# Lakonik/SSDNeRF

Hardware: NVIDIA H100
Metric: rays/sec (128^2 render) & DDIM triplanes/sec (higher is better)
Workload: dtype fp16 tensor-core UNet (fp32 accumulate), fp32 renderer

## Files before the change

include/ssdnerf_b200.h:

```cpp
#ifndef SSDNERF_B200_H_
#define SSDNERF_B200_H_

#include <stdint.h>
#include <stddef.h>

#ifdef __cplusplus
extern "C" {
#endif

#define SSDNERF_API __attribute__((visibility("default")))

#define SSDNERF_OK 0
#define SSDNERF_ERR_CUDA (-1)
#define SSDNERF_ERR_ARG (-2)
#define SSDNERF_ERR_ARCH (-3)

SSDNERF_API const char* ssdnerf_last_error(void);
SSDNERF_API int ssdnerf_version(void);
SSDNERF_API int ssdnerf_compiled_arch(void);
SSDNERF_API unsigned long long ssdnerf_launch_count(void);

SSDNERF_API int ssdnerf_near_far_from_aabb(const float* rays_o, const float* rays_d, const float* aabb, uint32_t N, float min_near,
                               float* nears, float* fars, void* stream);
SSDNERF_API int ssdnerf_sph_from_ray(const float* rays_o, const float* rays_d, float radius, uint32_t N, float* coords, void* stream);
// ... 101 lines not shown
SSDNERF_API int ssdnerf_unpack_plane_grads(const float* grad_planes, const float* code, float reg_coef, uint32_t B, uint32_t Hp, uint32_t Wp,
                               int accumulate, float* grad_code, void* stream);
SSDNERF_API int ssdnerf_mse_render_loss(const float* image, const float* weights_sum, const float* target, uint64_t rays, float bg_color,
                            float coef_loss, float coef_grad, float* out_rgb , float* grad_image, float* grad_ws,
                            float* loss , void* stream);

SSDNERF_API size_t ssdnerf_density_workspace_bytes(uint32_t num_scenes, uint32_t grid_size);
SSDNERF_API int ssdnerf_density_update(int variant, const void* planes, uint32_t plane_h, uint32_t plane_w, const float* decoder_blob,
                           uint32_t num_scenes, uint32_t grid_size, float bound,
                           const float* jitter,
                           float decay, void* density_grid, int grid_is_half, void* workspace, void* stream);
SSDNERF_API int ssdnerf_density_pack(const void* density_grid, int grid_is_half, uint32_t num_scenes, uint32_t grid_size,
                         float density_thresh, uint8_t* bitfield, float* thresh_out ,
                         void* workspace, void* stream);

typedef struct ssdnerf_gemm_args {
    const void* a1; uint64_t a1_strides[3]; uint32_t k1;
    const void* a2; uint64_t a2_strides[3]; uint32_t k2;
    uint32_t d1, d2, d3, b1, b2, b3;
    uint32_t taps;
    const void* b; uint64_t b_strides[3]; uint32_t n, n_rows_b, bx2, bx3; uint32_t b_batched;
    uint32_t bn;
    float alpha;
    const float* bias_n;
    const void* residual;
    void* out; uint32_t out_f32; long long so1, so2, so3;
    float* qstats; uint32_t stats_hw;
    uint32_t algo;
    const int8_t* tap_offsets;
    uint32_t a_stride;
    uint32_t relu;
} ssdnerf_gemm_args;
SSDNERF_API int ssdnerf_gemm_f16(const ssdnerf_gemm_args* args, void* stream);

SSDNERF_API int ssdnerf_nchw_to_nhwc_f16(const float* x, uint32_t B, uint32_t C, uint32_t H, uint32_t W, uint32_t Cpad, void* out, void* stream);
SSDNERF_API int ssdnerf_gn_stats(const void* x1, uint32_t C1, const void* x2, uint32_t C2, uint32_t B, uint32_t HW, uint32_t groups,
                                 float* stats, void* stream);
SSDNERF_API int ssdnerf_gn_apply_q(const void* x1, uint32_t C1, const void* x2, uint32_t C2, uint32_t B, uint32_t HW, uint32_t groups,
                                   const float* q1, const float* q2, const float* gamma, const float* beta, const float* scale_shift,
                                   long long ss_batch_stride, float eps, int do_silu, void* out, void* stream);
SSDNERF_API int ssdnerf_gn_apply(const void* x1, uint32_t C1, const void* x2, uint32_t C2, uint32_t B, uint32_t HW, uint32_t groups,
                                 const float* stats, const float* gamma, const float* beta, const float* scale_shift,
                                 long long ss_batch_stride, float eps, int do_silu, void* out, void* stream);
SSDNERF_API int ssdnerf_flash_attn(const void* qkv, uint32_t B, uint32_t T, uint32_t heads, uint32_t ch, float scale, void* out, void* stream);
SSDNERF_API int ssdnerf_softmax_rows(const float* S, uint32_t rows, uint32_t T, void* P, void* stream);
SSDNERF_API int ssdnerf_transpose_v(const void* qkv, uint32_t B, uint32_t T, uint32_t heads, uint32_t ch, void* vt, void* stream);
SSDNERF_API int ssdnerf_ddim_update(float* x_t, const float* v, uint32_t B, uint32_t C, uint32_t H, uint32_t W, uint32_t Cv,
                                    const float* coef, const int* step_ptr, int clip, float clip_lo, float clip_hi, float* x0_out,
                                    void* next_in, uint32_t Cpad, void* stream);
SSDNERF_API int ssdnerf_ddpm_update(float* x_t, const float* v, uint32_t B, uint32_t C, uint32_t H, uint32_t W, uint32_t Cv,
                                    const float* coef, const int* step_ptr, const unsigned long long* seed_ptr, int clip, float clip_lo,
                                    float clip_hi, void* next_in, uint32_t Cpad, void* stream);
SSDNERF_API int ssdnerf_step_counter(int* step_ptr, int value, int set, void* stream);
SSDNERF_API int ssdnerf_select_row(const float* table, uint32_t row_elems, const int* step_ptr, float* dst, uint32_t copies, void* stream);

typedef struct ssdnerf_gn_bwd_args {
    const void* x1; uint32_t C1;
    const void* x2; uint32_t C2;
    uint32_t B, HW, groups;
    const float* stats; const float* stats2; int quad_stats;
    const float* gamma; const float* beta;
    const float* scale_shift; long long ss_batch_stride;
    float eps; int do_silu;
    const void* dy;
    const void* add;
    float* group_sums;
// ... 157 lines not shown
```

ssdnerf_b200/csrc/conv_row2.cu:

```cuda
#include "common.cuh"
#include "tc_common.cuh"
#include "conv_row_epilogue.cuh"
#include "../../include/ssdnerf_b200.h"
#include <cuda_fp16.h>

namespace ssdnerf {
using namespace tc;

constexpr int kRwThreads = 384;
constexpr int kRwRowSlot = 17 * 1024;
constexpr int kRwBSlot = kRwN * 128;
constexpr int kRwRows = 6, kRwBStages = 6;
constexpr size_t kRwSmem = (size_t)kRwRows * kRwRowSlot + (size_t)kRwBStages * kRwBSlot + 1024  + 256  +
                           256  + 512 ;

struct ConvRowParams {
    uint32_t B, H;
    const __half* x1; uint32_t C1;
    const __half* x2; uint32_t C2;
    long long xs1[3], xs2[3];
    const float* bias;
    const __half* residual;
    __half* out;
    float* qstats;
};

__global__ void __launch_bounds__(kRwThreads, 1)
k_conv_row2(const __grid_constant__ CUtensorMap mapB, const ConvRowParams p) {
    extern __shared__ uint8_t smem_raw[];
    uint8_t* smem = reinterpret_cast<uint8_t*>(((uintptr_t)smem_raw + 1023) & ~(uintptr_t)1023);
    uint8_t* sR = smem;
    uint8_t* sB = smem + kRwRows * kRwRowSlot;
    uint64_t* fullR = reinterpret_cast<uint64_t*>(sB + kRwBStages * kRwBSlot);
    uint64_t* emptyR = fullR + kRwRows;
    uint64_t* fullB = emptyR + kRwRows;
    uint64_t* emptyB = fullB + kRwBStages;
    float* qacc = reinterpret_cast<float*>(reinterpret_cast<uint8_t*>(fullR) + 256);
    float* sbias = qacc + 64;

    const int warp = threadIdx.x >> 5, lane = threadIdx.x & 31, wg = warp >> 2;
    const uint32_t tiles_per_img = p.H / 2, total_tiles = p.B * tiles_per_img;
    const uint32_t kc1 = p.C1 / 64, KC = (p.C1 + p.C2) / 64;
    const uint32_t tile0 = blockIdx.x, tstep = gridDim.x;
    const uint32_t my_tiles = tile0 < total_tiles ? (total_tiles - tile0 + tstep - 1) / tstep : 0;

    if (threadIdx.x == 0) {
        prefetch_tmap(&mapB);
        for (int i = 0; i < kRwRows; ++i) { mbar_init(&fullR[i], 4); mbar_init(&emptyR[i], 8); }
        for (int i = 0; i < kRwBStages; ++i) { mbar_init(&fullB[i], 1); mbar_init(&emptyB[i], 8); }
        fence_mbar_init();
    }
    for (int i = threadIdx.x; i < 64; i += kRwThreads) qacc[i] = 0.0f;
    for (int i = threadIdx.x; i < kRwN; i += kRwThreads) sbias[i] = p.bias ? __ldg(p.bias + i) : 0.0f;
    __syncthreads();
    pdl_trigger();
    pdl_wait();

    if (wg == 2) {
        setmaxnreg_dec<120>();
        const uint32_t lt = threadIdx.x - 256u;
        const uint32_t c8 = lt & 7u, p0 = lt >> 3;
        uint32_t idx = 0;
        for (uint32_t tile = tile0; tile < total_tiles; tile += tstep) {
            const uint32_t b = tile / tiles_per_img, y0 = (tile - b * tiles_per_img) * 2;
            for (uint32_t j = 0; j < KC; ++j) {
                const bool first = j < kc1;
                const __half* src = first ? p.x1 : p.x2;
                const long long xs0 = first ? p.xs1[0] : p.xs2[0], xs1 = first ? p.xs1[1] : p.xs2[1], xs2 = first ? p.xs1[2] : p.xs2[2];
                const uint32_t cl = (first ? j : j - kc1) * 64u + c8 * 8u;
                for (uint32_t r = 0; r < 4; ++r) {
                    const int y = (int)(y0 + r) - 1;
                    const bool row_ok = y >= 0 && y < (int)p.H;
                    const __half* rowp = src + (long long)b * xs2 + (long long)(row_ok ? y : 0) * xs1 + cl;
                    uint4 v[9];
#pragma unroll
                    for (int n = 0; n < 9; ++n) {
                        const int x = (int)(p0 + 16u * n) - 1;
                        v[n] = (row_ok && (unsigned)x < (unsigned)kRwW) ? __ldg(reinterpret_cast<const uint4*>(rowp + (long long)x * xs0))
                                                                       : make_uint4(0, 0, 0, 0);
                    }
                    const uint32_t slot = idx % kRwRows;
                    mbar_wait(&emptyR[slot], ((idx / kRwRows) & 1u) ^ 1u);
                    const uint32_t dst = smem_u32(sR + slot * kRwRowSlot);
#pragma unroll
                    for (int n = 0; n < 9; ++n) {
                        const uint32_t px = p0 + 16u * n;
                        if (px >= 130u) continue;
                        sts128(dst + px * 128u + ((c8 ^ (px & 7u)) << 4), v[n]);
                    }
                    __syncwarp();
                    if (lane == 0) mbar_arrive(&fullR[slot]);
                    ++idx;
                }
            }
        }
    } else {
        setmaxnreg_inc<192>();
        const uint32_t a = (uint32_t)wg, wq = (uint32_t)warp & 3u, cq = (uint32_t)lane & 3u;
        const uint32_t steps_per_tile = KC * 9u, total_steps = my_tiles * steps_per_tile;
        auto issue_w = [&](uint32_t L) {
            const uint32_t s = L % kRwBStages;
            if (L >= (uint32_t)kRwBStages) mbar_wait(&emptyB[s], ((L / kRwBStages) - 1u) & 1u);
            mbar_expect_tx(&fullB[s], (uint32_t)kRwBSlot);
            const uint32_t rem = L % steps_per_tile;
            tma_load_4d(sB + s * kRwBSlot, &mapB, &fullB[s], (int)((rem / 9u) * 64u), 0, (int)(rem % 9u), 0);
        };
        if (threadIdx.x == 0)
            for (uint32_t L = 0; L < total_steps && L < (uint32_t)kRwBStages; ++L) issue_w(L);
        auto release_row = [&](uint32_t ring) { if (lane == 0) mbar_arrive(&emptyR[ring % kRwRows]); };
        uint32_t m = 0, ridx = 0;
        const uint32_t lrow = wq * 16u + ((uint32_t)lane & 15u);
        const uint32_t lk = (uint32_t)lane >> 4;
// ... 48 lines not shown
#pragma unroll
                for (int h = 0; h < 2; ++h) {
#pragma unroll
                    for (int hh = 0; hh < 2; ++hh) {
                        const size_t o = (pix0 + 64u * h + wq * 16u + ((uint32_t)lane >> 2) + 8u * hh) * kRwN + ch;
                        float v0 = (h ? acc1 : acc0)[4 * i + 2 * hh] + b0, v1 = (h ? acc1 : acc0)[4 * i + 2 * hh + 1] + b1;
                        if (p.residual) { const float2 r = __half22float2(*reinterpret_cast<const __half2*>(p.residual + o)); v0 += r.x; v1 += r.y; }
                        *reinterpret_cast<__half2*>(p.out + o) = __floats2half2_rn(v0, v1);
                        su += v0 + v1; sq = fmaf(v0, v0, fmaf(v1, v1, sq));
                    }
                }
                if (p.qstats) {
                    frag_quad_reduce(su, sq);
                    if ((lane & ~2) == 0) { float* qa = qacc + (2 * i + (lane >> 1)) * 2; atomicAdd(qa, su); atomicAdd(qa + 1, sq); }
                }
            }
            if (p.qstats) {
                asm volatile("bar.sync 1, 256;" ::: "memory");
                if (threadIdx.x < 64) {
                    const float val = qacc[threadIdx.x];
                    if (val != 0.0f) atomicAdd(p.qstats + (size_t)b * 64 + threadIdx.x, val);
                    qacc[threadIdx.x] = 0.0f;
                }
                asm volatile("bar.sync 1, 256;" ::: "memory");
            }
        }
    }
    __syncthreads();
}

int make_map_4d_box(CUtensorMap* m, const void* base, uint64_t K, uint64_t e1, uint64_t e2, uint64_t e3, uint64_t s1, uint64_t s2, uint64_t s3,
                    uint32_t x1, uint32_t x2, uint32_t x3);

static int launch_row2(const CUtensorMap& mB, const ConvRowParams& p, int sms, cudaStream_t stream) {
    static DeviceOnce attr;
    if (attr.first()) {
        SSDNERF_CUDA_OK(cudaFuncSetAttribute(k_conv_row2, cudaFuncAttributeMaxDynamicSharedMemorySize, (int)kRwSmem));
    }
    const uint32_t total = p.B * (p.H / 2);
    SSDNERF_CUDA_OK(launch_pdl(k_conv_row2, dim3(total < (uint32_t)sms ? total : (uint32_t)sms), dim3(kRwThreads), kRwSmem, stream, mB, p));
    SSDNERF_LAUNCH_OK();
    return 0;
}

int conv_row2_launch(const ssdnerf_gemm_args* a, int sms, cudaStream_t stream) {
    if (((uintptr_t)a->a1 & 15u) || ((a->a1_strides[0] | a->a1_strides[1] | a->a1_strides[2]) & 15u) ||
        (a->a2 && (((uintptr_t)a->a2 & 15u) || ((a->a2_strides[0] | a->a2_strides[1] | a->a2_strides[2]) & 15u))) ||
        ((uintptr_t)a->out & 3u) || ((uintptr_t)a->residual & 3u))
        return set_error_msg(SSDNERF_ERR_ARG, "gemm: row-pair convolution needs 16-byte aligned inputs and strides, 4-byte aligned output / residual");
    ConvRowParams p{};
    p.B = a->d3; p.H = a->d2;
    p.x1 = (const __half*)a->a1; p.C1 = a->k1;
    p.x2 = (const __half*)a->a2; p.C2 = a->a2 ? a->k2 : 0;
    for (int i = 0; i < 3; ++i) { p.xs1[i] = (long long)(a->a1_strides[i] / 2); p.xs2[i] = a->a2 ? (long long)(a->a2_strides[i] / 2) : 0; }
    p.bias = a->bias_n; p.residual = (const __half*)a->residual; p.out = (__half*)a->out; p.qstats = a->qstats;
    const uint64_t ktot = (uint64_t)a->k1 + (a->a2 ? a->k2 : 0);
    CUtensorMap mB;
    if (int e = make_map_4d_box(&mB, a->b, ktot, a->n_rows_b ? a->n_rows_b : a->n, a->bx2 ? a->bx2 : 1, a->bx3 ? a->bx3 : 1, a->b_strides[0],
                                a->b_strides[1], a->b_strides[2], kRwN, 1, 1)) return e;
    return launch_row2(mB, p, sms, stream);
}

}
```

ssdnerf_b200/csrc/gemm_tc.cu:

```cuda
#include "common.cuh"
#include "tc_common.cuh"
#include "conv_row_epilogue.cuh"
#include "../../include/ssdnerf_b200.h"
#include <cuda_fp16.h>
#include <cstdio>

namespace ssdnerf {
using namespace tc;

constexpr int kGemmThreads = 384;
constexpr int kMaxBiasN = 2048;
constexpr int kBM = 128, kBK = 64;
constexpr int kABytes = kBM * kBK * 2;

struct GemmParams {
    uint32_t b1, b2, b3;
    uint32_t d1, d2, d3;
    uint32_t T1, T2, T3;
    uint32_t tiles_n;
    uint32_t taps;
    int8_t tap_ox[9], tap_oy[9];
    uint32_t a_stride;
    uint32_t kc1, kc2;
    uint32_t n_valid;
// ... 212 lines not shown
        cudaDriverEntryPointQueryResult qres;
        if (cudaGetDriverEntryPoint("cuTensorMapEncodeTiled", &p, cudaEnableDefault, &qres) != cudaSuccess || !p) return nullptr;
        fn = (PFN_encodeTiled)p;
    }
    return fn;
}

static int make_map_4d(CUtensorMap* m, const void* base, uint64_t K, uint64_t e1, uint64_t e2, uint64_t e3, uint64_t s1, uint64_t s2,
                       uint64_t s3, uint32_t x1, uint32_t x2, uint32_t x3, uint32_t trav = 1) {
    PFN_encodeTiled enc = get_encode();
    if (!enc) return set_error_msg(SSDNERF_ERR_CUDA, "cuTensorMapEncodeTiled entry point not found");
    if (((uintptr_t)base & 15u) || (s1 & 15u) || (s2 & 15u) || (s3 & 15u))
        return set_error_msg(SSDNERF_ERR_ARG, "gemm: TMA operands need 16-byte aligned base and strides");
    cuuint64_t dims[4] = {K, e1, e2, e3};
    cuuint64_t strides[3] = {s1, s2, s3};
    cuuint32_t box[4] = {64, x1 * trav, x2 * trav, x3};
    cuuint32_t estr[4] = {1, trav, trav, 1};
    const CUresult r = enc(m, CU_TENSOR_MAP_DATA_TYPE_FLOAT16, 4, const_cast<void*>(base), dims, strides, box, estr,
                           CU_TENSOR_MAP_INTERLEAVE_NONE, CU_TENSOR_MAP_SWIZZLE_128B, CU_TENSOR_MAP_L2_PROMOTION_L2_256B,
                           CU_TENSOR_MAP_FLOAT_OOB_FILL_NONE);
    if (r != CUDA_SUCCESS) {
        char buf[200];
        snprintf(buf, sizeof(buf), "cuTensorMapEncodeTiled failed (%d): dims {%llu,%llu,%llu,%llu} box {64,%u,%u,%u}", (int)r,
                 (unsigned long long)K, (unsigned long long)e1, (unsigned long long)e2, (unsigned long long)e3, x1, x2, x3);
        return set_error_msg(SSDNERF_ERR_CUDA, buf);
    }
    return 0;
}

int make_map_4d_box(CUtensorMap* m, const void* base, uint64_t K, uint64_t e1, uint64_t e2, uint64_t e3, uint64_t s1, uint64_t s2, uint64_t s3,
                    uint32_t x1, uint32_t x2, uint32_t x3) {
    return make_map_4d(m, base, K, e1, e2, e3, s1, s2, s3, x1, x2, x3);
}
int conv_row2_launch(const ssdnerf_gemm_args* a, int sms, cudaStream_t stream);

template <int BN, bool KT = false, bool RELU = false>
static int launch_gemm(const CUtensorMap& mA1, const CUtensorMap& mA2, const CUtensorMap& mB, const GemmParams& p, int sms,
                       cudaStream_t stream) {
    using Cfg = GemmCfg<BN>;
    static DeviceOnce attr;
    if (attr.first()) {
        SSDNERF_CUDA_OK(cudaFuncSetAttribute(k_gemm_tc<BN, KT, RELU>, cudaFuncAttributeMaxDynamicSharedMemorySize, (int)Cfg::kSmem));
    }
    const uint32_t total = p.T1 * p.T2 * p.T3 * p.tiles_n;
    cudaLaunchConfig_t cfg{};
    cfg.gridDim = dim3(total < (uint32_t)sms ? total : (uint32_t)sms);
    cfg.blockDim = dim3(kGemmThreads);
    cfg.dynamicSmemBytes = Cfg::kSmem;
    cfg.stream = stream;
    cudaLaunchAttribute at[1];
    at[0].id = cudaLaunchAttributeProgrammaticStreamSerialization;
    at[0].val.programmaticStreamSerializationAllowed = pdl_enabled() ? 1 : 0;
    cfg.attrs = at; cfg.numAttrs = 1;
    SSDNERF_CUDA_OK(cudaLaunchKernelEx(&cfg, k_gemm_tc<BN, KT, RELU>, mA1, mA2, mB, p));
    SSDNERF_LAUNCH_OK();
    return 0;
}

}

using namespace ssdnerf;

extern "C" int ssdnerf_gemm_f16(const ssdnerf_gemm_args* a, void* stream_) {
    cudaStream_t stream = (cudaStream_t)stream_;
    if (!a || !a->a1 || !a->b || !a->out) return set_error_msg(SSDNERF_ERR_ARG, "gemm: a1, b and out are required");
    const bool kt = a->algo == 3;
    if (kt) {
        if (a->k1 == 0 || a->k1 % 8 || (a->a2 && (a->k2 == 0 || a->k2 % 8)))
            return set_error_msg(SSDNERF_ERR_ARG, "gemm (narrow): K extents must be multiples of 8");
    } else if (a->k1 == 0 || a->k1 % 64 || a->k2 % 64) {
        return set_error_msg(SSDNERF_ERR_ARG, "gemm: K extents must be multiples of 64");
    }
    if (a->b1 * a->b2 * a->b3 != 128) return set_error_msg(SSDNERF_ERR_ARG, "gemm: b1*b2*b3 must be 128");
    if (a->taps < 1 || a->taps > 9) return set_error_msg(SSDNERF_ERR_ARG, "gemm: taps must be in [1, 9]");
    if (a->taps != 1 && a->taps != 9 && !a->tap_offsets) return set_error_msg(SSDNERF_ERR_ARG, "gemm: taps other than 1 / 9 need tap_offsets");
    if (a->taps > 1 && a->b_batched) return set_error_msg(SSDNERF_ERR_ARG, "gemm: conv taps and batched B are exclusive");
    if (a->a_stride > 2) return set_error_msg(SSDNERF_ERR_ARG, "gemm: a_stride must be 0 / 1 / 2");
    const uint32_t a_stride = a->a_stride == 2 ? 2u : 1u;
    if (a_stride == 2 && (a->b1 * 2 > 256 || a->b2 * 2 > 256)) return set_error_msg(SSDNERF_ERR_ARG, "gemm: stride-2 boxes exceed the 256-element TMA limit");
    if (a->n == 0 || a->d1 == 0 || a->d2 == 0 || a->d3 == 0) return 0;
    int dev = 0, sms = 0;
    SSDNERF_CUDA_OK(cudaGetDevice(&dev));
    SSDNERF_CUDA_OK(cudaDeviceGetAttribute(&sms, cudaDevAttrMultiProcessorCount, dev));
    if (a->algo != 1 && !kt && !a->relu && a->taps == 9 && !a->tap_offsets && a_stride == 1 && a->d1 == 128 && a->b1 == 128 && a->b2 == 1 && a->b3 == 1 && a->n == 128 && !a->out_f32 && !a->b_batched &&
        (a->d2 % 2) == 0 && a->alpha == 1.0f && (a->bn == 0 || a->bn == 128) && a->so1 == 128 && a->so2 == 128 * 128 &&
        a->so3 == (long long)a->d2 * 128 * 128 && (!a->qstats || a->stats_hw == 0) && (a->n_rows_b == 0 || a->n_rows_b >= 128))
        return ssdnerf::conv_row2_launch(a, sms, stream);
    if (a->algo == 2) return set_error_msg(SSDNERF_ERR_ARG, "gemm: algo 2 (row-pair convolution) needs taps 9, 128-pixel rows, 128 output channels, fp16 output");
    int bn = (int)a->bn;
    if (kt) {
        const int cand[6] = {256, 160, 80, 48, 40, 16};
        if (a->relu) {
            if (bn && bn != 16) return set_error_msg(SSDNERF_ERR_ARG, "gemm (narrow): relu needs bn 0 or 16");
            bn = 16;
        } else if (bn) {
            bool ok = false;
            for (int c : cand) ok |= c == bn;
            if (!ok) return set_error_msg(SSDNERF_ERR_ARG, "gemm (narrow): bn must be 16, 40, 48, 80, 160 or 256");
        } else {
            for (int c : cand) if (a->n % (uint32_t)c == 0) { bn = c; break; }
            if (!bn) {
                uint32_t best = 0xFFFFFFFFu;
                for (int c : cand) { const uint32_t w = div_up(a->n, (uint32_t)c) * (uint32_t)c; if (w < best) { best = w; bn = c; } }
            }
        }
    } else if (!bn) {
        const uint32_t tiles_m = div_up(a->d1, a->b1) * div_up(a->d2, a->b2) * div_up(a->d3, a->b3);
        double best = 1e30;
        const int cand[3] = {256, 128, 64};
        const double eff[3] = {1.0, 0.80, 0.50};
        for (int i = 0; i < 3; ++i) {
            if (cand[i] > 64 && (uint32_t)cand[i] / 2 >= a->n) continue;
            const uint32_t tiles = tiles_m * div_up(a->n, (uint32_t)cand[i]);
            const double t = (double)div_up(tiles, (uint32_t)sms) * cand[i] / eff[i];
            if (t < best) { best = t; bn = cand[i]; }
        }
    }
    if (!kt && bn != 64 && bn != 128 && bn != 256) return set_error_msg(SSDNERF_ERR_ARG, "gemm: bn must be 64, 128 or 256");

    GemmParams p{};
// ... 54 lines not shown
```

ssdnerf_b200/csrc/unet_glue.cu:

```cuda
#include "common.cuh"
#include "../../include/ssdnerf_b200.h"

namespace ssdnerf {

__device__ __forceinline__ void h8_to_f(const uint4& v, float* f) {
    const __half2* h = reinterpret_cast<const __half2*>(&v);
#pragma unroll
    for (int i = 0; i < 4; ++i) { const float2 t = __half22float2(h[i]); f[2 * i] = t.x; f[2 * i + 1] = t.y; }
}
__device__ __forceinline__ uint4 f_to_h8(const float* f) {
    uint4 o;
    __half2* h = reinterpret_cast<__half2*>(&o);
#pragma unroll
    for (int i = 0; i < 4; ++i) h[i] = __floats2half2_rn(f[2 * i], f[2 * i + 1]);
    return o;
}

__global__ void k_nchw_to_nhwc(const float* __restrict__ x, uint32_t B, uint32_t C, uint32_t HW, uint32_t Cpad, __half* __restrict__ out) {
    pdl_trigger();
    pdl_wait();
    const size_t i = threadIdx.x + (size_t)blockIdx.x * blockDim.x;
    const uint32_t cv = Cpad / 8;
    if (i >= (size_t)B * HW * cv) return;
    const uint32_t v = (uint32_t)(i % cv);
    const size_t bp = i / cv;
    const uint32_t pix = (uint32_t)(bp % HW), b = (uint32_t)(bp / HW);
    float f[8];
#pragma unroll
    for (int k = 0; k < 8; ++k) {
        const uint32_t c = v * 8 + k;
        f[k] = c < C ? __ldg(x + ((size_t)b * C + c) * HW + pix) : 0.0f;
    }
    reinterpret_cast<uint4*>(out)[i] = f_to_h8(f);
}

__global__ void __launch_bounds__(256) k_gn_stats(const __half* __restrict__ x1, uint32_t C1, const __half* __restrict__ x2, uint32_t C2,
                                                  uint32_t HW, uint32_t groups, uint32_t pix_per_block, float* __restrict__ stats) {
    pdl_trigger();
    pdl_wait();
    extern __shared__ float sm[];
    const uint32_t C = C1 + C2, cv = C / 8, cv1 = C1 / 8;
    const uint32_t b = blockIdx.y;
    for (uint32_t i = threadIdx.x; i < 2 * C; i += blockDim.x) sm[i] = 0.0f;
    __syncthreads();
    const uint32_t p0 = blockIdx.x * pix_per_block, p1 = min(p0 + pix_per_block, HW);
    {
        const uint32_t v = threadIdx.x % cv, lane_p = threadIdx.x / cv, pstep = blockDim.x / cv;
        float s[8], q[8];
#pragma unroll
// ... 25 lines not shown
    __syncthreads();
    const uint32_t cpg = C / groups;
    for (uint32_t g = threadIdx.x; g < groups; g += blockDim.x) {
        float s = 0.0f, q = 0.0f;
        for (uint32_t c = g * cpg; c < (g + 1) * cpg; ++c) { s += sm[c]; q += sm[C + c]; }
        atomicAdd(stats + ((size_t)b * groups + g) * 2, s);
        atomicAdd(stats + ((size_t)b * groups + g) * 2 + 1, q);
    }
}

__global__ void __launch_bounds__(256) k_gn_apply(const __half* __restrict__ x1, uint32_t C1, const __half* __restrict__ x2, uint32_t C2,
                                                  uint32_t HW, uint32_t groups, uint32_t pix_per_block, const float* __restrict__ stats,
                                                  const float* __restrict__ stats2, int quad_stats, const float* __restrict__ gamma, const float* __restrict__ beta,
                                                  const float* __restrict__ scale_shift, long long ss_batch_stride, float eps, int do_silu,
                                                  __half* __restrict__ out) {
    pdl_trigger();
    pdl_wait();
    const uint32_t C = C1 + C2, cv = C / 8, cv1 = C1 / 8;
    const uint32_t b = blockIdx.y;
    const uint32_t v = threadIdx.x % cv, lane_p = threadIdx.x / cv, pstep = blockDim.x / cv;
    const uint32_t cpg = C / groups;
    const float inv_n = 1.0f / ((float)HW * (float)cpg);
    const float* ss = scale_shift ? scale_shift + (size_t)b * ss_batch_stride : nullptr;
    float ga[8], be[8], sc[8], sh[8];
#pragma unroll
    for (int k = 0; k < 8; ++k) {
        const uint32_t c = v * 8 + k;
        ga[k] = __ldg(gamma + c); be[k] = __ldg(beta + c);
        sc[k] = ss ? 1.0f + __ldg(ss + c) : 1.0f; sh[k] = ss ? __ldg(ss + C + c) : 0.0f;
    }
    __shared__ float2 s_mr[64];
    if (threadIdx.x < groups) {
        const uint32_t g = threadIdx.x;
        float sm = 0.0f, sq = 0.0f;
        if (!quad_stats) {
            sm = __ldg(stats + ((size_t)b * groups + g) * 2); sq = __ldg(stats + ((size_t)b * groups + g) * 2 + 1);
        } else {
            const uint32_t q1n = C1 / 4, q2n = C2 / 4, nq = cpg / 4;
            for (uint32_t i = 0; i < nq; ++i) {
                const uint32_t qi = g * nq + i;
                const float2 t = __ldg(reinterpret_cast<const float2*>(qi < q1n ? stats + ((size_t)b * q1n + qi) * 2
                                                                                  : stats2 + ((size_t)b * q2n + (qi - q1n)) * 2));
                sm += t.x; sq += t.y;
            }
        }
        const float mean = sm * inv_n;
        s_mr[g] = make_float2(mean, rsqrtf(fmaxf(sq * inv_n - mean * mean, 0.0f) + eps));
    }
    __syncthreads();
    float a[8], bb[8];
#pragma unroll
    for (int k = 0; k < 8; ++k) {
        const float2 mr = s_mr[(v * 8 + k) / cpg];
        const float ak = mr.y * ga[k];
        const float bk = be[k] - mr.x * ak;
        a[k] = ak * sc[k]; bb[k] = fmaf(bk, sc[k], sh[k]);
    }
    const __half* src = v < cv1 ? x1 + (size_t)b * HW * C1 + v * 8 : x2 + (size_t)b * HW * C2 + (v - cv1) * 8;
    const uint32_t cs = v < cv1 ? C1 : C2;
    __half* dst = out + (size_t)b * HW * C + v * 8;
    const uint32_t p0 = blockIdx.x * pix_per_block, p1 = min(p0 + pix_per_block, HW);
    auto emit = [&](const uint4& r, uint32_t p) {
        float f[8];
        h8_to_f(r, f);
#pragma unroll
        for (int k = 0; k < 8; ++k) { float y = fmaf(f[k], a[k], bb[k]); f[k] = do_silu ? silu_f(y) : y; }
        *reinterpret_cast<uint4*>(dst + (size_t)p * C) = f_to_h8(f);
    };
    uint32_t p = p0 + lane_p;
    for (; p + 3 * pstep < p1; p += 4 * pstep) {
        uint4 r[4];
#pragma unroll
        for (int u = 0; u < 4; ++u) r[u] = __ldg(reinterpret_cast<const uint4*>(src + (size_t)(p + u * pstep) * cs));
#pragma unroll
        for (int u = 0; u < 4; ++u) emit(r[u], p + u * pstep);
    }
    for (; p < p1; p += pstep) emit(__ldg(reinterpret_cast<const uint4*>(src + (size_t)p * cs)), p);
}

__global__ void __launch_bounds__(256) k_softmax_rows(const float* __restrict__ S, uint32_t rows, uint32_t T, __half* __restrict__ P) {
    pdl_trigger();
    pdl_wait();
    const uint32_t warp = threadIdx.x >> 5, lane = threadIdx.x & 31;
    const uint32_t row = blockIdx.x * 8 + warp;
    if (row >= rows) return;
    const float4* src = reinterpret_cast<const float4*>(S + (size_t)row * T);
    const uint32_t nv = T / 4;
    float m = -INFINITY;
    for (uint32_t i = lane; i < nv; i += 32) { const float4 v = __ldg(src + i); m = fmaxf(m, fmaxf(fmaxf(v.x, v.y), fmaxf(v.z, v.w))); }
#pragma unroll
    for (int o = 16; o > 0; o >>= 1) m = fmaxf(m, __shfl_xor_sync(0xffffffffu, m, o));
    float sum = 0.0f;
    for (uint32_t i = lane; i < nv; i += 32) { const float4 v = __ldg(src + i); sum += __expf(v.x - m) + __expf(v.y - m) + __expf(v.z - m) + __expf(v.w - m); }
#pragma unroll
    for (int o = 16; o > 0; o >>= 1) sum += __shfl_xor_sync(0xffffffffu, sum, o);
    const float inv = 1.0f / sum;
    __half2* dst = reinterpret_cast<__half2*>(P + (size_t)row * T);
    for (uint32_t i = lane; i < nv; i += 32) {
        const float4 v = __ldg(src + i);
        dst[2 * i] = __floats2half2_rn(__expf(v.x - m) * inv, __expf(v.y - m) * inv);
        dst[2 * i + 1] = __floats2half2_rn(__expf(v.z - m) * inv, __expf(v.w - m) * inv);
// ... 187 lines not shown
```

ssdnerf_b200/unet.py:

```python
import math
from copy import deepcopy

import torch
import torch.nn as nn

from . import _lib as N
from . import unet_ops as U
from .registry import MODULES


_GN_GROUPS = [32]


def _gn(c):
    return nn.GroupNorm(_GN_GROUPS[0], c, eps=1e-5)


class _ResBlockParams(nn.Module):

    def __init__(self, cin, cout, emb_ch, dropout=0.0):
        super().__init__()
        self.conv_1 = nn.Sequential(_gn(cin), nn.SiLU(), nn.Conv2d(cin, cout, 3, padding=1))
        self.norm_with_embedding = nn.Module()
        self.norm_with_embedding.norm = _gn(cout)
# ... 331 lines not shown
        L, s = N.lib(), N.stream_ptr()
        ss = None
        if ss_off is not None:
            ss = N.c_void_p(self.ss_cur.data_ptr() + 4 * ss_off)
        if ((C1 + C2) // G) % 4 != 0 or q1 is None or (x2 is not None and q2 is None):
            self._legacy_idx += 1
            st = self._q(('legacy', self._legacy_idx), G * 4)
            N.check(L.ssdnerf_gn_stats(N.ptr(x1), N.c_u32(C1), N.ptr(x2), N.c_u32(C2), N.c_u32(B), N.c_u32(H * W), N.c_u32(G), N.ptr(st), s))
            N.check(L.ssdnerf_gn_apply(N.ptr(x1), N.c_u32(C1), N.ptr(x2), N.c_u32(C2), N.c_u32(B), N.c_u32(H * W), N.c_u32(G), N.ptr(st),
                                       N.ptr(gamma), N.ptr(beta), ss, N.c_longlong(self.ss_total), N.c_f32(1e-5), N.c_int(int(silu)),
                                       N.ptr(out), s))
            self._last_stats = (False, st, None)
            return out
        self._last_stats = (True, q1, q2)
        N.check(L.ssdnerf_gn_apply_q(N.ptr(x1), N.c_u32(C1), N.ptr(x2), N.c_u32(C2), N.c_u32(B), N.c_u32(H * W), N.c_u32(G), N.ptr(q1),
                                     N.ptr(q2), N.ptr(gamma), N.ptr(beta), ss, N.c_longlong(self.ss_total), N.c_f32(1e-5),
                                     N.c_int(int(silu)), N.ptr(out), s))
        return out

    def _res(self, d, x, skip, tag):
        (x, qx), (sk, qs) = x, (skip if skip is not None else (None, None))
        B, H, W, _ = x.shape
        cin, cout = d['cin'], d['cout']
        nw = self.narrow
        if 'ws' in d:
            sc = U.conv3x3_f16(x, d['ws'].unsqueeze(0), cout, bias=d['wsb'], x2=sk, taps=1, out=self._buf(('sc', H, cout), (B, H, W, cout)),
                               narrow=nw)
        else:
            if sk is not None:
                raise NotImplementedError('ResBlock with a skip concat but no shortcut convolution (cin + skip == cout) is not built')
            sc = x
        qh1 = self._q(('h1', tag), cout)
        qo = self._q(('res_out', tag), cout)
        a = self._gn(x, qx, sk, qs, d['g1'], d['b1'], self._buf(('a', H, cin), (B, H, W, cin)), True)
        st1 = self._last_stats
        h1 = U.conv3x3_f16(a, d['w1'], cout, bias=d['c1b'], out=self._buf(('h1', tag) if self.saving else ('h1', H, cout), (B, H, W, cout)),
                           qstats=qh1, narrow=nw)
        a2 = self._gn(h1, qh1, None, None, d['g2'], d['b2'], self._buf(('a2', H, cout), (B, H, W, cout)), True, self.ss_offsets[d['idx']])
        st2 = self._last_stats
        if self.saving:
            self._dropout(a2, d['idx'])
        out = U.conv3x3_f16(a2, d['w2'], cout, bias=d['c2b'], residual=sc, out=self._buf(('res_out', tag), (B, H, W, cout)), qstats=qo,
                            narrow=nw)
        if self.saving:
            self.tape.append(dict(kind='res', d=d, x=x, sk=sk, st1=st1, h1=h1, st2=st2, out=out, tag=tag))
        return out, qo

    def _attn(self, d, x, tag):
        x, qx = x
        B, H, W, c = x.shape
        T, heads = H * W, d['heads']
        ch = c // heads
        L, s = N.lib(), N.stream_ptr()
        xn = self._gn(x, qx, None, None, d['g'], d['b'], self._buf(('xn', T, c), (B, H, W, c)), False)
        st = self._last_stats
        qkv = U.linear_f16(xn.view(B * T, c), d['wqkv'], bias=d['bqkv'], n=3 * c,
                           out=self._buf(('qkv', tag) if self.saving else ('qkv', T, c), (B * T, 3 * c)), narrow=self.narrow)
        o = self._attn_core(qkv, B, T, c, heads, ('o', T, c))
        qo = self._q(('attn_out', tag), c) if T % 64 == 0 else None
        out = U.linear_f16(o.view(B * T, c), d['wproj'], bias=d['bproj'], residual=x.view(B * T, c), n=c,
                           out=self._buf(('attn_out', tag), (B * T, c)), qstats=qo, stats_hw=T, narrow=self.narrow).view(B, H, W, c)
        if self.saving:
            self.tape.append(dict(kind='attn', d=d, x=x, st=st, qkv=qkv.view(B, T, 3 * c), out=out, tag=tag))
        return out, qo

    def _attn_core(self, qkv, B, T, c, heads, out_key):
        ch = c // heads
        L, s = N.lib(), N.stream_ptr()
        if ch in (64, 128) and T % 64 == 0:
            return U.flash_attn(qkv.view(B, T, 3 * c), heads, 1.0 / math.sqrt(ch), out=self._buf(out_key, (B, T, c)))
        S = U.attn_scores(qkv.view(B, T, 3 * c), heads, scale=1.0 / math.sqrt(ch), out=self._buf(('S', T), (B, heads, T, T), torch.float32),
                          narrow=self.narrow)
        P = self._buf(('P', T), (B, heads, T, T))
        N.check(L.ssdnerf_softmax_rows(N.ptr(S), N.c_u32(B * heads * T), N.c_u32(T), N.ptr(P), s))
        vt = self._buf(('vt', T, c), (B, heads, ch, T))
        N.check(L.ssdnerf_transpose_v(N.ptr(qkv), N.c_u32(B), N.c_u32(T), N.c_u32(heads), N.c_u32(ch), N.ptr(vt), s))
# ... 252 lines not shown
```

ssdnerf_b200/unet_ops.py:

```python
import ctypes

import torch

from . import _lib as N

c_u64 = ctypes.c_uint64
c_ll = ctypes.c_longlong


class GemmArgs(ctypes.Structure):
    _fields_ = [
        ('a1', N.c_void_p), ('a1_strides', c_u64 * 3), ('k1', N.c_u32),
        ('a2', N.c_void_p), ('a2_strides', c_u64 * 3), ('k2', N.c_u32),
        ('d1', N.c_u32), ('d2', N.c_u32), ('d3', N.c_u32), ('b1', N.c_u32), ('b2', N.c_u32), ('b3', N.c_u32),
        ('taps', N.c_u32),
        ('b', N.c_void_p), ('b_strides', c_u64 * 3), ('n', N.c_u32), ('n_rows_b', N.c_u32), ('bx2', N.c_u32), ('bx3', N.c_u32),
        ('b_batched', N.c_u32),
        ('bn', N.c_u32), ('alpha', N.c_f32), ('bias_n', N.c_void_p), ('residual', N.c_void_p),
        ('out', N.c_void_p), ('out_f32', N.c_u32), ('so1', c_ll), ('so2', c_ll), ('so3', c_ll),
        ('qstats', N.c_void_p), ('stats_hw', N.c_u32), ('algo', N.c_u32),
        ('tap_offsets', N.c_void_p), ('a_stride', N.c_u32), ('relu', N.c_u32),
    ]


ALGO_NARROW = 3


def _launch(a):
    N.check(N.lib().ssdnerf_gemm_f16(ctypes.byref(a), N.stream_ptr()))


def _pad_rows(w, mult=64):
    n = w.shape[-2]
    pad = (-n) % mult
    if pad:
        w = torch.cat([w, w.new_zeros(*w.shape[:-2], pad, w.shape[-1])], dim=-2)
    return w


def pack_linear_weight(w, narrow=False):
    w = w.detach().reshape(w.shape[0], -1).half()
    assert w.shape[1] % (8 if narrow else 64) == 0, 'K must be a multiple of 64 (narrow: of 8)'
    return _pad_rows(w).contiguous()


def pack_conv_weight(w, cin_pad=None, narrow=False):
    cout, cin = w.shape[0], w.shape[1]
    m = 8 if narrow else 64
    cin_pad = cin_pad or ((cin + m - 1) // m * m)
    wp = w.detach().permute(2, 3, 0, 1).reshape(9, cout, cin).half()
    if cin_pad != cin:
        wp = torch.cat([wp, wp.new_zeros(9, cout, cin_pad - cin)], dim=-1)
    return _pad_rows(wp).contiguous()


# ... 18 lines not shown
    g.out, g.out_f32 = out.data_ptr(), int(out.dtype == torch.float32)
    g.so1, g.so2, g.so3 = out.stride(0), 0, 0
    if qstats is not None:
        g.qstats, g.stats_hw = qstats.data_ptr(), stats_hw
    if narrow:
        g.algo = ALGO_NARROW
    _launch(g)
    return out


def _conv_boxes(H, W, narrow=False):
    if narrow:
        return _conv_boxes_narrow(H, W)
    bw = min(W, 128)
    bh = min(H, 128 // bw)
    nb = 128 // (bw * bh)
    return bw, bh, nb


def _pow2_floor(v):
    return 1 << (max(int(v), 1).bit_length() - 1)


def _conv_boxes_narrow(H, W):
    bw = min(128, W & -W)
    bh = min(128 // bw, _pow2_floor(H))
    if 128 // (bw * bh) > 2:
        bw = min(128, 1 << (W - 1).bit_length())
        bh = min(128 // bw, 1 << (H - 1).bit_length())
    return bw, bh, 128 // (bw * bh)


def conv3x3_f16(x, wp, cout, bias=None, x2=None, residual=None, out=None, out_f32=False, taps=9, bn=0, qstats=None, algo=0, narrow=False,
                relu=False):
    N.require_cuda(x, wp)
    B, H, W, C1 = x.shape
    C2 = x2.shape[-1] if x2 is not None else 0
    assert x.is_contiguous() and (x2 is None or x2.is_contiguous())
    km = 8 if narrow else 64
    assert wp.shape[-1] == C1 + C2 and C1 % km == 0 and C2 % km == 0, (wp.shape, C1, C2)
    if narrow:
        algo = ALGO_NARROW
    if out is None:
        out = torch.empty(B, H, W, cout, dtype=torch.float32 if out_f32 else torch.float16, device=x.device)
    bw, bh, nb = _conv_boxes(H, W, narrow)
    g = GemmArgs()
    g.a1, g.k1 = x.data_ptr(), C1
    g.a1_strides = (c_u64 * 3)(C1 * 2, W * C1 * 2, H * W * C1 * 2)
    if x2 is not None:
        g.a2, g.k2 = x2.data_ptr(), C2
        g.a2_strides = (c_u64 * 3)(C2 * 2, W * C2 * 2, H * W * C2 * 2)
    g.d1, g.d2, g.d3, g.b1, g.b2, g.b3 = W, H, B, bw, bh, nb
    g.taps = taps
    ktot = C1 + C2
    rows = wp.shape[-2]
    g.b, g.n, g.n_rows_b, g.bx2, g.bx3 = wp.data_ptr(), cout, rows, taps, 1
    g.b_strides = (c_u64 * 3)(ktot * 2, rows * ktot * 2, taps * rows * ktot * 2)
    g.bn, g.alpha, g.algo = bn, 1.0, algo
    g.bias_n = bias.data_ptr() if bias is not None else None
    g.residual = residual.data_ptr() if residual is not None else None
    g.out, g.out_f32 = out.data_ptr(), int(out.dtype == torch.float32)
    co = out.shape[-1]
    g.so1, g.so2, g.so3 = co, W * co, H * W * co
    if qstats is not None:
        g.qstats, g.stats_hw = qstats.data_ptr(), 0
    g.relu = int(relu)
    _launch(g)
    return out


def conv3x3_s2_f16(x, wp, cout, bias=None, out=None, qstats=None, narrow=False):
    N.require_cuda(x, wp)
    B, H, W, C = x.shape
    assert x.is_contiguous() and H % 2 == 0 and W % 2 == 0 and wp.shape[-1] == C and C % (8 if narrow else 64) == 0
    Ho, Wo = H // 2, W // 2
    if out is None:
        out = torch.empty(B, Ho, Wo, cout, dtype=torch.float16, device=x.device)
    bw, bh, nb = _conv_boxes(Ho, Wo, narrow)
    g = GemmArgs()
    g.a1, g.k1 = x.data_ptr(), C
    g.a1_strides = (c_u64 * 3)(C * 2, W * C * 2, H * W * C * 2)
    g.d1, g.d2, g.d3, g.b1, g.b2, g.b3 = Wo, Ho, B, bw, bh, nb
    g.taps, g.a_stride = 9, 2
    rows = wp.shape[-2]
    g.b, g.n, g.n_rows_b, g.bx2, g.bx3 = wp.data_ptr(), cout, rows, 9, 1
    g.b_strides = (c_u64 * 3)(C * 2, rows * C * 2, 9 * rows * C * 2)
    g.bn, g.alpha, g.algo = 0, 1.0, ALGO_NARROW if narrow else 1
    g.bias_n = bias.data_ptr() if bias is not None else None
    g.out, g.out_f32 = out.data_ptr(), int(out.dtype == torch.float32)
    g.so1, g.so2, g.so3 = cout, Wo * cout, Ho * Wo * cout
    if qstats is not None:
        g.qstats, g.stats_hw = qstats.data_ptr(), 0
    _launch(g)
    return out


_UP_ROWS = {0: ((-1, (0,)), (0, (1, 2))), 1: ((0, (0, 1)), (1, (2,)))}


def pack_upconv_weight(w, narrow=False):
    w = w.detach().float()
# ... 247 lines not shown
```

Measured before the change: 97.93 million.

## Fuse GroupNorm+SiLU apply into the row-pair convolution loader

Adds a GroupNorm descriptor to the fp16 GEMM entry point. When it is given, the row-pair 3x3 conv's loader warps normalize, scale/shift and apply SiLU to each input vector before staging it in shared memory, so the resblock no longer writes and re-reads a separate normalized activation buffer. The unet glue routes the 128-wide, 128-channel resblocks through this path. The cost is extra per-channel coefficient loads and group-stat reductions inside the producer warps, which could slow the producer side of the pipeline.

```diff
diff --git a/include/ssdnerf_b200.h b/include/ssdnerf_b200.h
--- a/include/ssdnerf_b200.h
+++ b/include/ssdnerf_b200.h
@@ -157,6 +157,14 @@
     uint32_t relu;
 } ssdnerf_gemm_args;
 SSDNERF_API int ssdnerf_gemm_f16(const ssdnerf_gemm_args* args, void* stream);
+typedef struct ssdnerf_gn_desc {
+    const float* q1; const float* q2;
+    const float* gamma; const float* beta;
+    const float* scale_shift;
+    long long ss_batch_stride;
+    float eps; uint32_t groups;
+} ssdnerf_gn_desc;
+SSDNERF_API int ssdnerf_gemm_f16_gn(const ssdnerf_gemm_args* args, const ssdnerf_gn_desc* gn, void* stream);
 
 SSDNERF_API int ssdnerf_nchw_to_nhwc_f16(const float* x, uint32_t B, uint32_t C, uint32_t H, uint32_t W, uint32_t Cpad, void* out, void* stream);
 SSDNERF_API int ssdnerf_gn_stats(const void* x1, uint32_t C1, const void* x2, uint32_t C2, uint32_t B, uint32_t HW, uint32_t groups,
diff --git a/ssdnerf_b200/csrc/conv_row2.cu b/ssdnerf_b200/csrc/conv_row2.cu
--- a/ssdnerf_b200/csrc/conv_row2.cu
+++ b/ssdnerf_b200/csrc/conv_row2.cu
@@ -1,6 +1,7 @@
 #include "common.cuh"
 #include "tc_common.cuh"
 #include "conv_row_epilogue.cuh"
+#include "gn_apply.cuh"
 #include "../../include/ssdnerf_b200.h"
 #include <cuda_fp16.h>
 
@@ -23,8 +24,32 @@
     const __half* residual;
     __half* out;
     float* qstats;
+    const float* gq1; const float* gq2;
+    const float* gamma; const float* beta;
+    const float* ss; long long ss_stride;
+    float eps; uint32_t cpg;
 };
 
+__device__ __forceinline__ void loader_gn_coeffs(const ConvRowParams& p, uint32_t b, uint32_t c0, float* a, float* bb) {
+    const uint32_t C = p.C1 + p.C2, nq = p.cpg / 4;
+    const float* ss = p.ss ? p.ss + (size_t)b * p.ss_stride : nullptr;
+    float ga[8], be[8], sc[8], sh[8];
+#pragma unroll
+    for (int k = 0; k < 8; ++k) {
+        const uint32_t c = c0 + k;
+        ga[k] = __ldg(p.gamma + c); be[k] = __ldg(p.beta + c);
+        sc[k] = ss ? 1.0f + __ldg(ss + c) : 1.0f; sh[k] = ss ? __ldg(ss + C + c) : 0.0f;
+    }
+    const uint32_t g0 = c0 / p.cpg, g1 = (c0 + 7u) / p.cpg;
+    const float2 s0 = gn_quad_group_sums(p.gq1, p.gq2, p.C1 / 4, p.C2 / 4, b, g0, nq);
+    const float2 s1 = gn_quad_group_sums(p.gq1, p.gq2, p.C1 / 4, p.C2 / 4, b, g1, nq);
+    const float inv_n = 1.0f / ((float)(p.H * kRwW) * (float)p.cpg);
+    const float2 mr0 = gn_mean_rstd(s0, inv_n, p.eps), mr1 = gn_mean_rstd(s1, inv_n, p.eps);
+#pragma unroll
+    for (int k = 0; k < 8; ++k) gn_fold((c0 + k) / p.cpg == g0 ? mr0 : mr1, ga[k], be[k], sc[k], sh[k], a[k], bb[k]);
+}
+
+template <bool GN>
 __global__ void __launch_bounds__(kRwThreads, 1)
 k_conv_row2(const __grid_constant__ CUtensorMap mapB, const ConvRowParams p) {
     extern __shared__ uint8_t smem_raw[];
@@ -68,6 +93,8 @@
                 const __half* src = first ? p.x1 : p.x2;
                 const long long xs0 = first ? p.xs1[0] : p.xs2[0], xs1 = first ? p.xs1[1] : p.xs2[1], xs2 = first ? p.xs1[2] : p.xs2[2];
                 const uint32_t cl = (first ? j : j - kc1) * 64u + c8 * 8u;
+                float ga[8], gb[8];
+                if constexpr (GN) loader_gn_coeffs(p, b, j * 64u + c8 * 8u, ga, gb);
                 for (uint32_t r = 0; r < 4; ++r) {
                     const int y = (int)(y0 + r) - 1;
                     const bool row_ok = y >= 0 && y < (int)p.H;
@@ -78,6 +105,11 @@
                         const int x = (int)(p0 + 16u * n) - 1;
                         v[n] = (row_ok && (unsigned)x < (unsigned)kRwW) ? __ldg(reinterpret_cast<const uint4*>(rowp + (long long)x * xs0))
                                                                        : make_uint4(0, 0, 0, 0);
+                    }
+                    if constexpr (GN) {
+#pragma unroll
+                        for (int n = 0; n < 9; ++n)
+                            if (row_ok && (unsigned)((int)(p0 + 16u * n) - 1) < (unsigned)kRwW) v[n] = gn_transform_h8(v[n], ga, gb, true);
                     }
                     const uint32_t slot = idx % kRwRows;
                     mbar_wait(&emptyR[slot], ((idx / kRwRows) & 1u) ^ 1u);
@@ -192,18 +224,19 @@
 int make_map_4d_box(CUtensorMap* m, const void* base, uint64_t K, uint64_t e1, uint64_t e2, uint64_t e3, uint64_t s1, uint64_t s2, uint64_t s3,
                     uint32_t x1, uint32_t x2, uint32_t x3);
 
+template <bool GN>
 static int launch_row2(const CUtensorMap& mB, const ConvRowParams& p, int sms, cudaStream_t stream) {
     static DeviceOnce attr;
     if (attr.first()) {
-        SSDNERF_CUDA_OK(cudaFuncSetAttribute(k_conv_row2, cudaFuncAttributeMaxDynamicSharedMemorySize, (int)kRwSmem));
+        SSDNERF_CUDA_OK(cudaFuncSetAttribute(k_conv_row2<GN>, cudaFuncAttributeMaxDynamicSharedMemorySize, (int)kRwSmem));
     }
     const uint32_t total = p.B * (p.H / 2);
-    SSDNERF_CUDA_OK(launch_pdl(k_conv_row2, dim3(total < (uint32_t)sms ? total : (uint32_t)sms), dim3(kRwThreads), kRwSmem, stream, mB, p));
+    SSDNERF_CUDA_OK(launch_pdl(k_conv_row2<GN>, dim3(total < (uint32_t)sms ? total : (uint32_t)sms), dim3(kRwThreads), kRwSmem, stream, mB, p));
     SSDNERF_LAUNCH_OK();
     return 0;
 }
 
-int conv_row2_launch(const ssdnerf_gemm_args* a, int sms, cudaStream_t stream) {
+int conv_row2_launch(const ssdnerf_gemm_args* a, const ssdnerf_gn_desc* gn, int sms, cudaStream_t stream) {
     if (((uintptr_t)a->a1 & 15u) || ((a->a1_strides[0] | a->a1_strides[1] | a->a1_strides[2]) & 15u) ||
         (a->a2 && (((uintptr_t)a->a2 & 15u) || ((a->a2_strides[0] | a->a2_strides[1] | a->a2_strides[2]) & 15u))) ||
         ((uintptr_t)a->out & 3u) || ((uintptr_t)a->residual & 3u))
@@ -214,11 +247,15 @@
     p.x2 = (const __half*)a->a2; p.C2 = a->a2 ? a->k2 : 0;
     for (int i = 0; i < 3; ++i) { p.xs1[i] = (long long)(a->a1_strides[i] / 2); p.xs2[i] = a->a2 ? (long long)(a->a2_strides[i] / 2) : 0; }
     p.bias = a->bias_n; p.residual = (const __half*)a->residual; p.out = (__half*)a->out; p.qstats = a->qstats;
+    if (gn) {
+        p.gq1 = gn->q1; p.gq2 = a->a2 ? gn->q2 : nullptr; p.gamma = gn->gamma; p.beta = gn->beta;
+        p.ss = gn->scale_shift; p.ss_stride = gn->ss_batch_stride; p.eps = gn->eps; p.cpg = (p.C1 + p.C2) / gn->groups;
+    }
     const uint64_t ktot = (uint64_t)a->k1 + (a->a2 ? a->k2 : 0);
     CUtensorMap mB;
     if (int e = make_map_4d_box(&mB, a->b, ktot, a->n_rows_b ? a->n_rows_b : a->n, a->bx2 ? a->bx2 : 1, a->bx3 ? a->bx3 : 1, a->b_strides[0],
                                 a->b_strides[1], a->b_strides[2], kRwN, 1, 1)) return e;
-    return launch_row2(mB, p, sms, stream);
-}
-
-}
+    return gn ? launch_row2<true>(mB, p, sms, stream) : launch_row2<false>(mB, p, sms, stream);
+}
+
+}
diff --git a/ssdnerf_b200/csrc/gemm_tc.cu b/ssdnerf_b200/csrc/gemm_tc.cu
--- a/ssdnerf_b200/csrc/gemm_tc.cu
+++ b/ssdnerf_b200/csrc/gemm_tc.cu
@@ -268,7 +268,7 @@
                     uint32_t x1, uint32_t x2, uint32_t x3) {
     return make_map_4d(m, base, K, e1, e2, e3, s1, s2, s3, x1, x2, x3);
 }
-int conv_row2_launch(const ssdnerf_gemm_args* a, int sms, cudaStream_t stream);
+int conv_row2_launch(const ssdnerf_gemm_args* a, const ssdnerf_gn_desc* gn, int sms, cudaStream_t stream);
 
 template <int BN, bool KT = false, bool RELU = false>
 static int launch_gemm(const CUtensorMap& mA1, const CUtensorMap& mA2, const CUtensorMap& mB, const GemmParams& p, int sms,
@@ -297,9 +297,18 @@
 
 using namespace ssdnerf;
 
-extern "C" int ssdnerf_gemm_f16(const ssdnerf_gemm_args* a, void* stream_) {
+extern "C" int ssdnerf_gemm_f16(const ssdnerf_gemm_args* a, void* stream) { return ssdnerf_gemm_f16_gn(a, nullptr, stream); }
+
+extern "C" int ssdnerf_gemm_f16_gn(const ssdnerf_gemm_args* a, const ssdnerf_gn_desc* gn, void* stream_) {
     cudaStream_t stream = (cudaStream_t)stream_;
     if (!a || !a->a1 || !a->b || !a->out) return set_error_msg(SSDNERF_ERR_ARG, "gemm: a1, b and out are required");
+    if (gn) {
+        const uint32_t C = a->k1 + (a->a2 ? a->k2 : 0);
+        if (!gn->q1 || (a->a2 && !gn->q2) || !gn->gamma || !gn->beta)
+            return set_error_msg(SSDNERF_ERR_ARG, "gemm: a GroupNorm descriptor needs quad statistics of every source, gamma and beta");
+        if (gn->groups == 0 || C % gn->groups || (C / gn->groups) % 4)
+            return set_error_msg(SSDNERF_ERR_ARG, "gemm: GroupNorm groups must be a whole number of 4-channel quads");
+    }
     const bool kt = a->algo == 3;
     if (kt) {
         if (a->k1 == 0 || a->k1 % 8 || (a->a2 && (a->k2 == 0 || a->k2 % 8)))
@@ -321,7 +330,8 @@
     if (a->algo != 1 && !kt && !a->relu && a->taps == 9 && !a->tap_offsets && a_stride == 1 && a->d1 == 128 && a->b1 == 128 && a->b2 == 1 && a->b3 == 1 && a->n == 128 && !a->out_f32 && !a->b_batched &&
         (a->d2 % 2) == 0 && a->alpha == 1.0f && (a->bn == 0 || a->bn == 128) && a->so1 == 128 && a->so2 == 128 * 128 &&
         a->so3 == (long long)a->d2 * 128 * 128 && (!a->qstats || a->stats_hw == 0) && (a->n_rows_b == 0 || a->n_rows_b >= 128))
-        return ssdnerf::conv_row2_launch(a, sms, stream);
+        return ssdnerf::conv_row2_launch(a, gn, sms, stream);
+    if (gn) return set_error_msg(SSDNERF_ERR_ARG, "gemm: a GroupNorm descriptor needs the row-pair convolution (taps 9, 128-pixel rows, 128 output channels, fp16 output)");
     if (a->algo == 2) return set_error_msg(SSDNERF_ERR_ARG, "gemm: algo 2 (row-pair convolution) needs taps 9, 128-pixel rows, 128 output channels, fp16 output");
     int bn = (int)a->bn;
     if (kt) {
diff --git a/ssdnerf_b200/csrc/gn_apply.cuh b/ssdnerf_b200/csrc/gn_apply.cuh
--- /dev/null
+++ b/ssdnerf_b200/csrc/gn_apply.cuh
@@ -0,0 +1,56 @@
+#pragma once
+#include "common.cuh"
+
+namespace ssdnerf {
+
+__device__ __forceinline__ void h8_to_f(const uint4& v, float* f) {
+    const __half2* h = reinterpret_cast<const __half2*>(&v);
+#pragma unroll
+    for (int i = 0; i < 4; ++i) { const float2 t = __half22float2(h[i]); f[2 * i] = t.x; f[2 * i + 1] = t.y; }
+}
+__device__ __forceinline__ uint4 f_to_h8(const float* f) {
+    uint4 o;
+    __half2* h = reinterpret_cast<__half2*>(&o);
+#pragma unroll
+    for (int i = 0; i < 4; ++i) h[i] = __floats2half2_rn(f[2 * i], f[2 * i + 1]);
+    return o;
+}
+
+__device__ __forceinline__ float2 gn_quad_group_sums(const float* __restrict__ q1, const float* __restrict__ q2, uint32_t q1n, uint32_t q2n,
+                                                     uint32_t b, uint32_t g, uint32_t nq) {
+    float sm = 0.0f, sq = 0.0f;
+    for (uint32_t i0 = 0; i0 < nq; i0 += 4) {
+        float2 t[4];
+#pragma unroll
+        for (uint32_t u = 0; u < 4; ++u) {
+            const uint32_t qi = g * nq + i0 + u;
+            t[u] = i0 + u < nq ? __ldg(reinterpret_cast<const float2*>(qi < q1n ? q1 + ((size_t)b * q1n + qi) * 2 : q2 + ((size_t)b * q2n + (qi - q1n)) * 2))
+                               : make_float2(0.0f, 0.0f);
+        }
+#pragma unroll
+        for (uint32_t u = 0; u < 4; ++u)
+            if (i0 + u < nq) { sm += t[u].x; sq += t[u].y; }
+    }
+    return make_float2(sm, sq);
+}
+
+__device__ __forceinline__ float2 gn_mean_rstd(float2 sums, float inv_n, float eps) {
+    const float mean = sums.x * inv_n;
+    return make_float2(mean, rsqrtf(fmaxf(sums.y * inv_n - mean * mean, 0.0f) + eps));
+}
+
+__device__ __forceinline__ void gn_fold(float2 mr, float ga, float be, float sc, float sh, float& a, float& b) {
+    const float ak = mr.y * ga;
+    const float bk = be - mr.x * ak;
+    a = ak * sc; b = fmaf(bk, sc, sh);
+}
+
+__device__ __forceinline__ uint4 gn_transform_h8(const uint4& r, const float* a, const float* b, bool silu) {
+    float f[8];
+    h8_to_f(r, f);
+#pragma unroll
+    for (int k = 0; k < 8; ++k) { float y = fmaf(f[k], a[k], b[k]); f[k] = silu ? silu_f(y) : y; }
+    return f_to_h8(f);
+}
+
+}
diff --git a/ssdnerf_b200/csrc/unet_glue.cu b/ssdnerf_b200/csrc/unet_glue.cu
--- a/ssdnerf_b200/csrc/unet_glue.cu
+++ b/ssdnerf_b200/csrc/unet_glue.cu
@@ -1,20 +1,8 @@
 #include "common.cuh"
+#include "gn_apply.cuh"
 #include "../../include/ssdnerf_b200.h"
 
 namespace ssdnerf {
-
-__device__ __forceinline__ void h8_to_f(const uint4& v, float* f) {
-    const __half2* h = reinterpret_cast<const __half2*>(&v);
-#pragma unroll
-    for (int i = 0; i < 4; ++i) { const float2 t = __half22float2(h[i]); f[2 * i] = t.x; f[2 * i + 1] = t.y; }
-}
-__device__ __forceinline__ uint4 f_to_h8(const float* f) {
-    uint4 o;
-    __half2* h = reinterpret_cast<__half2*>(&o);
-#pragma unroll
-    for (int i = 0; i < 4; ++i) h[i] = __floats2half2_rn(f[2 * i], f[2 * i + 1]);
-    return o;
-}
 
 __global__ void k_nchw_to_nhwc(const float* __restrict__ x, uint32_t B, uint32_t C, uint32_t HW, uint32_t Cpad, __half* __restrict__ out) {
     pdl_trigger();
@@ -106,41 +94,20 @@
     __shared__ float2 s_mr[64];
     if (threadIdx.x < groups) {
         const uint32_t g = threadIdx.x;
-        float sm = 0.0f, sq = 0.0f;
-        if (!quad_stats) {
-            sm = __ldg(stats + ((size_t)b * groups + g) * 2); sq = __ldg(stats + ((size_t)b * groups + g) * 2 + 1);
-        } else {
-            const uint32_t q1n = C1 / 4, q2n = C2 / 4, nq = cpg / 4;
-            for (uint32_t i = 0; i < nq; ++i) {
-                const uint32_t qi = g * nq + i;
-                const float2 t = __ldg(reinterpret_cast<const float2*>(qi < q1n ? stats + ((size_t)b * q1n + qi) * 2
-                                                                                  : stats2 + ((size_t)b * q2n + (qi - q1n)) * 2));
-                sm += t.x; sq += t.y;
-            }
-        }
-        const float mean = sm * inv_n;
-        s_mr[g] = make_float2(mean, rsqrtf(fmaxf(sq * inv_n - mean * mean, 0.0f) + eps));
+        float2 sums;
+        if (!quad_stats) sums = make_float2(__ldg(stats + ((size_t)b * groups + g) * 2), __ldg(stats + ((size_t)b * groups + g) * 2 + 1));
+        else sums = gn_quad_group_sums(stats, stats2, C1 / 4, C2 / 4, b, g, cpg / 4);
+        s_mr[g] = gn_mean_rstd(sums, inv_n, eps);
     }
     __syncthreads();
     float a[8], bb[8];
 #pragma unroll
-    for (int k = 0; k < 8; ++k) {
-        const float2 mr = s_mr[(v * 8 + k) / cpg];
-        const float ak = mr.y * ga[k];
-        const float bk = be[k] - mr.x * ak;
-        a[k] = ak * sc[k]; bb[k] = fmaf(bk, sc[k], sh[k]);
-    }
+    for (int k = 0; k < 8; ++k) gn_fold(s_mr[(v * 8 + k) / cpg], ga[k], be[k], sc[k], sh[k], a[k], bb[k]);
     const __half* src = v < cv1 ? x1 + (size_t)b * HW * C1 + v * 8 : x2 + (size_t)b * HW * C2 + (v - cv1) * 8;
     const uint32_t cs = v < cv1 ? C1 : C2;
     __half* dst = out + (size_t)b * HW * C + v * 8;
     const uint32_t p0 = blockIdx.x * pix_per_block, p1 = min(p0 + pix_per_block, HW);
-    auto emit = [&](const uint4& r, uint32_t p) {
-        float f[8];
-        h8_to_f(r, f);
-#pragma unroll
-        for (int k = 0; k < 8; ++k) { float y = fmaf(f[k], a[k], bb[k]); f[k] = do_silu ? silu_f(y) : y; }
-        *reinterpret_cast<uint4*>(dst + (size_t)p * C) = f_to_h8(f);
-    };
+    auto emit = [&](const uint4& r, uint32_t p) { *reinterpret_cast<uint4*>(dst + (size_t)p * C) = gn_transform_h8(r, a, bb, do_silu); };
     uint32_t p = p0 + lane_p;
     for (; p + 3 * pstep < p1; p += 4 * pstep) {
         uint4 r[4];
diff --git a/ssdnerf_b200/unet.py b/ssdnerf_b200/unet.py
--- a/ssdnerf_b200/unet.py
+++ b/ssdnerf_b200/unet.py
@@ -387,16 +387,29 @@
             sc = x
         qh1 = self._q(('h1', tag), cout)
         qo = self._q(('res_out', tag), cout)
-        a = self._gn(x, qx, sk, qs, d['g1'], d['b1'], self._buf(('a', H, cin), (B, H, W, cin)), True)
-        st1 = self._last_stats
-        h1 = U.conv3x3_f16(a, d['w1'], cout, bias=d['c1b'], out=self._buf(('h1', tag) if self.saving else ('h1', H, cout), (B, H, W, cout)),
-                           qstats=qh1, narrow=nw)
-        a2 = self._gn(h1, qh1, None, None, d['g2'], d['b2'], self._buf(('a2', H, cout), (B, H, W, cout)), True, self.ss_offsets[d['idx']])
-        st2 = self._last_stats
-        if self.saving:
-            self._dropout(a2, d['idx'])
-        out = U.conv3x3_f16(a2, d['w2'], cout, bias=d['c2b'], residual=sc, out=self._buf(('res_out', tag), (B, H, W, cout)), qstats=qo,
-                            narrow=nw)
+        G = self.groups
+        row_pair = U.row_pair_conv(H, W, cout, nw)
+        h1_out = self._buf(('h1', tag) if self.saving else ('h1', H, cout), (B, H, W, cout))
+        if row_pair and qx is not None and (sk is None or qs is not None) and (cin // G) % 4 == 0:
+            st1 = (True, qx, qs)
+            h1 = U.conv3x3_f16(x, d['w1'], cout, bias=d['c1b'], x2=sk, out=h1_out, qstats=qh1,
+                               gn=U.gn_desc(qx, qs, d['g1'], d['b1'], G))
+        else:
+            a = self._gn(x, qx, sk, qs, d['g1'], d['b1'], self._buf(('a', H, cin), (B, H, W, cin)), True)
+            st1 = self._last_stats
+            h1 = U.conv3x3_f16(a, d['w1'], cout, bias=d['c1b'], out=h1_out, qstats=qh1, narrow=nw)
+        ss_off = self.ss_offsets[d['idx']]
+        res_out = self._buf(('res_out', tag), (B, H, W, cout))
+        if row_pair and qh1 is not None and (cout // G) % 4 == 0 and not (self.saving and self._drop_seed is not None):
+            st2 = (True, qh1, None)
+            out = U.conv3x3_f16(h1, d['w2'], cout, bias=d['c2b'], residual=sc, out=res_out, qstats=qo,
+                                gn=U.gn_desc(qh1, None, d['g2'], d['b2'], G, self.ss_cur.data_ptr() + 4 * ss_off, self.ss_total))
+        else:
+            a2 = self._gn(h1, qh1, None, None, d['g2'], d['b2'], self._buf(('a2', H, cout), (B, H, W, cout)), True, ss_off)
+            st2 = self._last_stats
+            if self.saving:
+                self._dropout(a2, d['idx'])
+            out = U.conv3x3_f16(a2, d['w2'], cout, bias=d['c2b'], residual=sc, out=res_out, qstats=qo, narrow=nw)
         if self.saving:
             self.tape.append(dict(kind='res', d=d, x=x, sk=sk, st1=st1, h1=h1, st2=st2, out=out, tag=tag))
         return out, qo
diff --git a/ssdnerf_b200/unet_ops.py b/ssdnerf_b200/unet_ops.py
--- a/ssdnerf_b200/unet_ops.py
+++ b/ssdnerf_b200/unet_ops.py
@@ -21,6 +21,21 @@
         ('qstats', N.c_void_p), ('stats_hw', N.c_u32), ('algo', N.c_u32),
         ('tap_offsets', N.c_void_p), ('a_stride', N.c_u32), ('relu', N.c_u32),
     ]
+
+
+class GnDesc(ctypes.Structure):
+    _fields_ = [
+        ('q1', N.c_void_p), ('q2', N.c_void_p), ('gamma', N.c_void_p), ('beta', N.c_void_p),
+        ('scale_shift', N.c_void_p), ('ss_batch_stride', c_ll), ('eps', N.c_f32), ('groups', N.c_u32),
+    ]
+
+
+def gn_desc(q1, q2, gamma, beta, groups, scale_shift_addr=None, ss_batch_stride=0, eps=1e-5):
+    d = GnDesc()
+    d.q1, d.q2 = q1.data_ptr(), (q2.data_ptr() if q2 is not None else None)
+    d.gamma, d.beta = gamma.data_ptr(), beta.data_ptr()
+    d.scale_shift, d.ss_batch_stride, d.eps, d.groups = scale_shift_addr, ss_batch_stride, eps, groups
+    return d
 
 
 ALGO_NARROW = 3
@@ -105,7 +120,7 @@
 
 
 def conv3x3_f16(x, wp, cout, bias=None, x2=None, residual=None, out=None, out_f32=False, taps=9, bn=0, qstats=None, algo=0, narrow=False,
-                relu=False):
+                relu=False, gn=None):
     N.require_cuda(x, wp)
     B, H, W, C1 = x.shape
     C2 = x2.shape[-1] if x2 is not None else 0
@@ -138,8 +153,15 @@
     if qstats is not None:
         g.qstats, g.stats_hw = qstats.data_ptr(), 0
     g.relu = int(relu)
-    _launch(g)
-    return out
+    if gn is not None:
+        N.check(N.lib().ssdnerf_gemm_f16_gn(ctypes.byref(g), ctypes.byref(gn), N.stream_ptr()))
+    else:
+        _launch(g)
+    return out
+
+
+def row_pair_conv(H, W, cout, narrow=False):
+    return not narrow and W == 128 and cout == 128 and H % 2 == 0
 
 
 def conv3x3_s2_f16(x, wp, cout, bias=None, out=None, qstats=None, narrow=False):
```

Result: no change. 97.91 million (median of 6 runs) (-0.0%).
